# vfdev-5/interpolate-antialiasing

Hardware: AMD Instinct MI355X
Metric: Mpix/s (input pixels) antialiased bilinear 438x906->196x320, uint8 channels_last, PIL-exact (higher is better)
Workload: dtype u8; 1 GPU; uint8 channels_last [1024,3,438,906]->[196,320] bilinear antialias per GPU (BASELINE configs[1] batched), Pillow-exact integer arithmetic; batch_per_gpu=1024, global_batch=1024, variant=fused_u8_nhwc_pil_v3, parallelism=batch-shard x1, lib=interpolate_antialiasing_amd/csrc/libaa_interp.so

## Files before the change

### include/aa_interp.h

```cpp
#ifndef AA_INTERP_H
#define AA_INTERP_H

#include <stddef.h>
#include <stdint.h>

#ifdef __cplusplus
extern "C" {
#endif

#define AA_INTERP_ABI_VERSION 3

typedef void *aa_stream_t;

enum aa_status {
  AA_OK = 0,
  AA_ERR_BAD_FILTER = -1,
  AA_ERR_BAD_DTYPE = -2,
  AA_ERR_BAD_LAYOUT = -3,
  AA_ERR_BAD_SHAPE = -4,
  AA_ERR_NULL = -5,
  AA_ERR_WORKSPACE = -6,
  AA_ERR_KSIZE = -7,
  AA_ERR_HIP = -8,
  AA_ERR_NO_DEVICE = -9,
// ... 94 lines not shown
  int32_t out_layout;
  int32_t normalize;
  float mean[4];
  float std[4];
  uint32_t flags;
} aa_convert;
size_t aa_workspace_bytes_u8_to_f32(int layout, int64_t N, int64_t C, int64_t H, int64_t W, const aa_axis *ax_h, const aa_axis *ax_w,
                                    const aa_convert *cv);
int aa_resample_fwd_u8_to_f32(const void *in_dev, void *out_dev, void *workspace_dev, size_t workspace_bytes, int layout,
                              int64_t N, int64_t C, int64_t H, int64_t W, const aa_axis *ax_h, const aa_axis *ax_w,
                              const aa_convert *cv, aa_stream_t stream);

int aa_resample_bwd(const void *grad_out_dev, void *grad_in_dev, void *workspace_dev, size_t workspace_bytes, int dtype,
                    int layout, int64_t N, int64_t C, int64_t H, int64_t W, const aa_axis *tr_h, const aa_axis *tr_w,
                    aa_stream_t stream);
int aa_resample_bwd_atomic(const void *grad_out_dev, void *grad_in_dev, void *workspace_dev, size_t workspace_bytes,
                           int dtype, int layout, int64_t N, int64_t C, int64_t H, int64_t W, const aa_axis *ax_h,
                           const aa_axis *ax_w, aa_stream_t stream);
size_t aa_workspace_bytes_bwd(int dtype, int layout, int64_t N, int64_t C, int64_t H, int64_t W, int64_t oH, int64_t oW);

int aa_resample_axis_fwd(const void *in_dev, void *out_dev, int dtype, int64_t outer, int64_t in_size, int64_t inner,
                         const aa_axis *ax, aa_stream_t stream);

int aa_reduce_u8(const void *in_dev, void *out_dev, int layout, int64_t N, int64_t C, int64_t H, int64_t W, const int64_t *in_strides,
                 const int64_t *box, int fx, int fy, aa_stream_t stream);
int aa_premultiply_u8(const void *src_dev, void *dst_dev, int layout, int64_t N, int64_t C, int64_t H, int64_t W, aa_stream_t stream);
int aa_unpremultiply_u8(void *img_dev, int layout, int64_t N, int64_t C, int64_t H, int64_t W, aa_stream_t stream);

#define AA_MANY_FLIP_X 1
typedef struct aa_many_image {
  const void *data_dev;
  int64_t H, W;
  int64_t stride_row, stride_px, stride_ch;
  double box[4];
  int32_t has_box;
  int32_t flags;
} aa_many_image;
size_t aa_many_desc_bytes(int64_t n);
int aa_many_plan(int filter, int layout, int64_t n, int64_t C, int64_t oH, int64_t oW, const aa_many_image *images, void *desc_host,
                 size_t desc_bytes, size_t *workspace_bytes);
int aa_resample_many_u8(const void *desc_host, const void *desc_dev, int64_t n, int64_t C, int64_t oH, int64_t oW, int layout, void *out_dev,
                        void *workspace_dev, size_t workspace_bytes, aa_stream_t stream);
int aa_resample_many_u8_to_float(const void *desc_host, const void *desc_dev, int64_t n, int64_t C, int64_t oH, int64_t oW, int layout,
                                 void *out_dev, void *workspace_dev, size_t workspace_bytes, const aa_convert *cv, aa_stream_t stream);

int aa_probe_copy(const void *src_dev, void *dst_dev, size_t bytes, int form, aa_stream_t stream);

int aa_set_fused(int enabled);

int aa_set_store_form(int form);

int aa_set_plane_groups(int enabled);

const char *aa_last_variant(void);

#ifdef __cplusplus
}
#endif
#endif
```

### interpolate_antialiasing_amd/_lib.py

```python
from __future__ import annotations

import collections
import ctypes
import os

_HERE = os.path.dirname(os.path.abspath(__file__))
LIB_PATH = os.environ.get("AA_INTERP_LIB") or os.path.join(_HERE, "csrc", "libaa_interp.so")
HEADER_PATH = os.path.join(os.path.dirname(_HERE), "include", "aa_interp.h")

AA_OK = 0
FILTER_LINEAR, FILTER_CUBIC, FILTER_BOX, FILTER_HAMMING, FILTER_LANCZOS = 0, 1, 2, 3, 4
Filter = collections.namedtuple("Filter", "id name aliases support op")
FILTERS = (Filter(FILTER_LINEAR, "linear", ("bilinear",), 1.0, "linear"), Filter(FILTER_CUBIC, "cubic", ("bicubic",), 2.0, "cubic"),
           Filter(FILTER_BOX, "box", ("nearest",), 0.5, "nearest"), Filter(FILTER_HAMMING, "hamming", (), 1.0, "hamming"),
           Filter(FILTER_LANCZOS, "lanczos", (), 3.0, "lanczos"))
FILTER_NAMES = {f.id: f.name for f in FILTERS}


def by_filter_name(value) -> dict:
    return {n: value(f) for f in FILTERS for n in (f.name,) + f.aliases}


FILTER_IDS = by_filter_name(lambda f: f.id)
U8, F32, F64, F16, BF16 = 0, 1, 2, 3, 4
NCHW, NHWC = 0, 1
TABLE_PIL, TABLE_F32, TABLE_F64 = 0, 1, 2
ERR_BAD_DTYPE = -2
ERR_STRIDES = -10
FLAG_FAST = 1
FLAG_PREMUL_ALPHA = 2
FLAG_OUT_F16 = 4
FLAG_OUT_BF16 = 8

EXPORTS = (
    "aa_abi_version", "aa_strerror", "aa_device_count", "aa_table_ksize", "aa_table_bytes", "aa_table_build_bytes", "aa_table_build",
    "aa_table_transposed_ksize", "aa_table_transpose", "aa_table_query", "aa_table_query2", "aa_table_build2", "aa_workspace_bytes", "aa_resample_fwd",
    "aa_resample_bwd", "aa_resample_bwd_atomic", "aa_workspace_bytes_bwd", "aa_resample_axis_fwd", "aa_set_fused",
    "aa_last_variant", "aa_probe_copy", "aa_workspace_bytes_u8_to_f32", "aa_resample_fwd_u8_to_f32", "aa_set_store_form", "aa_set_plane_groups", "aa_resample_fwd_ex", "aa_resample_fwd_strided",
    "aa_workspace_bytes_ex", "aa_table_ksize_box", "aa_table_build_bytes_box", "aa_table_build_box", "aa_reduce_u8", "aa_premultiply_u8",
    "aa_unpremultiply_u8", "aa_many_desc_bytes", "aa_many_plan", "aa_resample_many_u8", "aa_resample_many_u8_to_float",
)


class TableHeader(ctypes.Structure):
    _fields_ = [
        ("magic", ctypes.c_int32), ("filter", ctypes.c_int32), ("kind", ctypes.c_int32), ("in_size", ctypes.c_int32),
        ("out_size", ctypes.c_int32), ("ksize", ctypes.c_int32), ("align_corners", ctypes.c_int32),
        ("max_taps", ctypes.c_int32), ("transposed", ctypes.c_int32), ("scatter_off", ctypes.c_int32),
        ("scatter_ksize", ctypes.c_int32), ("scatter_max", ctypes.c_int32), ("span64p1", ctypes.c_int32), ("span4p1", ctypes.c_int32), ("gather_off", ctypes.c_int32), ("reserved", ctypes.c_int32 * 1),
    ]


class Axis(ctypes.Structure):
    _fields_ = [
        ("table_dev", ctypes.c_void_p), ("in_size", ctypes.c_int32), ("out_size", ctypes.c_int32),
        ("ksize", ctypes.c_int32), ("max_taps", ctypes.c_int32), ("kind", ctypes.c_int32), ("filter", ctypes.c_int32),
        ("scatter_off", ctypes.c_int32), ("scatter_ksize", ctypes.c_int32), ("scatter_max", ctypes.c_int32),
        ("span64p1", ctypes.c_int32), ("span4p1", ctypes.c_int32), ("gather_off", ctypes.c_int32), ("reserved", ctypes.c_int32 * 2),
    ]


class Convert(ctypes.Structure):
    _fields_ = [("out_layout", ctypes.c_int32), ("normalize", ctypes.c_int32), ("mean", ctypes.c_float * 4),
                ("std", ctypes.c_float * 4), ("flags", ctypes.c_uint32)]


class ManyImage(ctypes.Structure):
    _fields_ = [("data_dev", ctypes.c_void_p), ("H", ctypes.c_int64), ("W", ctypes.c_int64), ("stride_row", ctypes.c_int64),
                ("stride_px", ctypes.c_int64), ("stride_ch", ctypes.c_int64), ("box", ctypes.c_double * 4), ("has_box", ctypes.c_int32),
                ("flags", ctypes.c_int32)]


class ManyHeader(ctypes.Structure):
    _fields_ = [("magic", ctypes.c_int32), ("n", ctypes.c_int32), ("C", ctypes.c_int32), ("oH", ctypes.c_int32), ("oW", ctypes.c_int32),
                ("filter", ctypes.c_int32), ("layout", ctypes.c_int32), ("reserved0", ctypes.c_int32), ("hunits", ctypes.c_int64),
                ("ws_bytes", ctypes.c_int64), ("reserved", ctypes.c_int64 * 2)]


class ManyItem(ctypes.Structure):
    _fields_ = [("src", ctypes.c_void_p), ("row_stride", ctypes.c_int64), ("plane_stride", ctypes.c_int64), ("tab_h", ctypes.c_int64),
                ("tab_w", ctypes.c_int64), ("inter", ctypes.c_int64), ("in0_h", ctypes.c_double), ("in1_h", ctypes.c_double),
                ("in0_w", ctypes.c_double), ("in1_w", ctypes.c_double), ("oy", ctypes.c_int32), ("hull_h", ctypes.c_int32),
                ("ox", ctypes.c_int32), ("hull_w", ctypes.c_int32), ("ksize_h", ctypes.c_int32), ("ksize_w", ctypes.c_int32),
                ("box_on", ctypes.c_int32), ("reserved", ctypes.c_int32)]


MANY_FLIP_X = 1
MANY_STRIP = 64


def many_desc_view(buf, n: int):
# ... 47 lines not shown
    L.aa_table_build2.restype = i32
    L.aa_workspace_bytes.argtypes = [i32, i32, i64, i64, i64, i64, i64, i64, ax, ax]
    L.aa_workspace_bytes.restype = sz
    L.aa_workspace_bytes_ex.argtypes = [i32, i32, i64, i64, i64, i64, i64, i64, ax, ax, ctypes.c_uint]
    L.aa_workspace_bytes_ex.restype = sz
    L.aa_resample_fwd.argtypes = [vp, vp, vp, sz, i32, i32, i64, i64, i64, i64, ax, ax, vp]
    L.aa_resample_fwd.restype = i32
    L.aa_resample_fwd_ex.argtypes = [vp, vp, vp, sz, i32, i32, i64, i64, i64, i64, ax, ax, ctypes.c_uint, vp]
    L.aa_resample_fwd_ex.restype = i32
    L.aa_resample_fwd_strided.argtypes = [vp, vp, i32, i32, i64, i64, i64, i64, ctypes.POINTER(ctypes.c_int64), ax, ax, ctypes.c_uint, vp]
    L.aa_resample_fwd_strided.restype = i32
    L.aa_resample_bwd.argtypes = [vp, vp, vp, sz, i32, i32, i64, i64, i64, i64, ax, ax, vp]
    L.aa_resample_bwd.restype = i32
    L.aa_resample_bwd_atomic.argtypes = [vp, vp, vp, sz, i32, i32, i64, i64, i64, i64, ax, ax, vp]
    L.aa_resample_bwd_atomic.restype = i32
    L.aa_workspace_bytes_bwd.argtypes = [i32, i32, i64, i64, i64, i64, i64, i64]
    L.aa_workspace_bytes_bwd.restype = sz
    L.aa_resample_axis_fwd.argtypes = [vp, vp, i32, i64, i64, i64, ax, vp]
    L.aa_resample_axis_fwd.restype = i32
    L.aa_last_variant.restype = ctypes.c_char_p
    cvp = ctypes.POINTER(Convert)
    L.aa_workspace_bytes_u8_to_f32.argtypes = [i32, i64, i64, i64, i64, ax, ax, cvp]
    L.aa_workspace_bytes_u8_to_f32.restype = sz
    L.aa_resample_fwd_u8_to_f32.argtypes = [vp, vp, vp, sz, i32, i64, i64, i64, i64, ax, ax, cvp, vp]
    L.aa_resample_fwd_u8_to_f32.restype = i32
    L.aa_probe_copy.argtypes = [vp, vp, sz, i32, vp]
    L.aa_probe_copy.restype = i32
    L.aa_table_ksize_box.argtypes = [i32, i32, i64, i64, dbl, dbl]
    L.aa_table_ksize_box.restype = i32
    L.aa_table_build_bytes_box.argtypes = [i32, i32, i64, i64, dbl, dbl]
    L.aa_table_build_bytes_box.restype = sz
    L.aa_table_build_box.argtypes = [i32, i32, i64, i64, i64, dbl, dbl, vp, sz, i64, i64, i64, dbl, dbl, vp, sz, vp]
    L.aa_table_build_box.restype = i32
    L.aa_reduce_u8.argtypes = [vp, vp, i32, i64, i64, i64, i64, ctypes.POINTER(ctypes.c_int64), ctypes.POINTER(ctypes.c_int64), i32, i32, vp]
    L.aa_reduce_u8.restype = i32
    L.aa_premultiply_u8.argtypes = [vp, vp, i32, i64, i64, i64, i64, vp]
    L.aa_premultiply_u8.restype = i32
    L.aa_unpremultiply_u8.argtypes = [vp, i32, i64, i64, i64, i64, vp]
    L.aa_unpremultiply_u8.restype = i32
    L.aa_many_desc_bytes.argtypes = [i64]
    L.aa_many_desc_bytes.restype = sz
    L.aa_many_plan.argtypes = [i32, i32, i64, i64, i64, i64, ctypes.POINTER(ManyImage), vp, sz, ctypes.POINTER(sz)]
    L.aa_many_plan.restype = i32
    L.aa_resample_many_u8.argtypes = [vp, vp, i64, i64, i64, i64, i32, vp, vp, sz, vp]
    L.aa_resample_many_u8.restype = i32
    L.aa_resample_many_u8_to_float.argtypes = [vp, vp, i64, i64, i64, i64, i32, vp, vp, sz, cvp, vp]
    L.aa_resample_many_u8_to_float.restype = i32
    L.aa_set_fused.argtypes = [i32]
    L.aa_set_fused.restype = i32
    L.aa_set_store_form.argtypes = [i32]
    L.aa_set_store_form.restype = i32
    L.aa_set_plane_groups.argtypes = [i32]
    L.aa_set_plane_groups.restype = i32
    if L.aa_abi_version() != 3:
        raise AAInterpError("libaa_interp.so ABI version mismatch")
    _lib = L
    return L


def strerror(rc: int) -> str:
    return load().aa_strerror(rc).decode()


def check(rc: int, what: str = "") -> None:
    if rc < 0:
        msg = f"{what}: {strerror(rc)} (aa_status {rc})" if what else f"{strerror(rc)} (aa_status {rc})"
        if rc == ERR_BAD_DTYPE:
            raise NotImplementedError(msg)
        raise AAInterpError(msg)


fused_epoch = 0


def set_fused(enabled: int) -> int:
    global fused_epoch
    fused_epoch += 1
    return int(load().aa_set_fused(int(enabled)))


def set_store_form(form: int) -> int:
    return int(load().aa_set_store_form(int(form)))


def set_plane_groups(enabled: int) -> int:
    return int(load().aa_set_plane_groups(int(enabled)))


def last_variant() -> str:
    return load().aa_last_variant().decode()


KERNEL_SOURCES = {
    "fused_u8_nhwc_pil_v3": ("aa_fused_u8_v3_impl.h", "aa_fused_u8_v3.hip", "aa_fused_u8_v3_unit.hip", "aa_fused_u8_v3_list.h", "aa_common.h"),
    "fused_u8_nhwc_pil": ("aa_fused_u8.hip", "aa_common.h"),
    "fused_u8_planar_pil_v3": ("aa_fused_u8_v3_impl.h", "aa_fused_u8_v3.hip", "aa_fused_u8_v3_unit.hip", "aa_fused_u8_v3_list.h", "aa_common.h"),
}


def source_fingerprint(variant: str):
    import hashlib

    names = KERNEL_SOURCES.get(variant)
    if not names:
        return None
    h = hashlib.sha256()
    for n in names:
        with open(os.path.join(_HERE, "csrc", n), "rb") as f:
            h.update(n.encode() + b"\0" + f.read())
    return h.hexdigest()[:12]
```

### interpolate_antialiasing_amd/csrc/aa_api.hip

```cpp

#include <math.h>
#include <string.h>

#include "aa_box.h"
#include "aa_many.h"
#include "aa_plan.h"
#include "aa_reduce.h"

int g_aa_store_form = -1;
int g_aa_plane_groups = 1;

namespace {

thread_local const char *g_last_variant = "none";
int g_fused_enabled = 1;

int interp_size_of(int filter) { return aa_filter_valid(filter) ? aa_filter_info(filter).interp_size : -1; }

double scale_for(int kind, int64_t in_size, int64_t out_size, int align_corners, double scale_opt) {
  if (kind == AA_TABLE_F32) {
    if (align_corners) return out_size > 1 ? (double)((float)(in_size - 1) / (float)(out_size - 1)) : 0.0;
    if (scale_opt > 0.) return (double)(float)(1.0 / scale_opt);
    return (double)((float)in_size / (float)out_size);
  }
  if (align_corners) return out_size > 1 ? (double)(in_size - 1) / (double)(out_size - 1) : 0.0;
  if (scale_opt > 0.) return 1.0 / scale_opt;
  return (double)in_size / (double)out_size;
}

int ksize_for(int filter, int kind, double scale) {
  const int interp_size = interp_size_of(filter);
  if (kind == AA_TABLE_PIL) {
    const double fs = aa_filter_info(filter).support;
    const double filterscale = scale < 1.0 ? 1.0 : scale;
    return (int)ceil(fs * filterscale) * 2 + 1;
  }
  if (kind == AA_TABLE_F32) {
    const float s = (float)scale;
    const float support = (s >= 1.0) ? (float)((interp_size * 0.5) * s) : (float)(interp_size * 0.5);
    return (int)ceilf(support) * 2 + 1;
  }
  const double support = (scale >= 1.0) ? (interp_size * 0.5) * scale : interp_size * 0.5;
  return (int)ceilf((float)support) * 2 + 1;
}

bool valid_kind(int kind) { return kind == AA_TABLE_PIL || kind == AA_TABLE_F32 || kind == AA_TABLE_F64; }

int check_axis(const aa_axis *a, int64_t in_size) {
  if (!a || !a->table_dev) return AA_ERR_NULL;
  if (a->in_size != in_size || a->out_size <= 0 || a->ksize <= 0) return AA_ERR_BAD_SHAPE;
  if (a->ksize > AA_MAX_KSIZE) return AA_ERR_KSIZE;
  if (!valid_kind(a->kind)) return AA_ERR_BAD_DTYPE;
  return AA_OK;
}

int check_dtype_kind(int dtype, int kh, int kw) {
  if (kh != kw) return AA_ERR_BAD_DTYPE;
  if (dtype == AA_F32 && kh == AA_TABLE_F32) return AA_OK;
  if (dtype == AA_F64 && kh == AA_TABLE_F64) return AA_OK;
  if (dtype == AA_U8 && (kh == AA_TABLE_PIL || kh == AA_TABLE_F32)) return AA_OK;
  if ((dtype == AA_F16 || dtype == AA_BF16) && kh == AA_TABLE_F32) return AA_OK;
  return AA_ERR_BAD_DTYPE;
}
// ... 550 lines not shown
    g_last_variant = "empty";
    return AA_OK;
  }
  if (!grad_out_dev || !grad_in_dev) return AA_ERR_NULL;
  const size_t need = aa_workspace_bytes_bwd(dtype, layout, N, C, H, W, ax_h->out_size, ax_w->out_size);
  if (!workspace_dev || workspace_bytes < need) return AA_ERR_WORKSPACE;
  AAProblem q = problem(dtype, layout, N, C, H, W, ax_h->out_size, ax_w->out_size, *ax_h, *ax_w, 0u);
  q.in = grad_out_dev; q.out = grad_in_dev; q.ws = workspace_dev; q.ws_bytes = workspace_bytes;
  q.stream = (hipStream_t)stream;
  rc = aa_launch_bwd_atomic(q);
  if (rc == AA_OK) g_last_variant = "bwd_scatter_atomics";
  return rc;
}

int aa_resample_axis_fwd(const void *in_dev, void *out_dev, int dtype, int64_t outer, int64_t in_size, int64_t inner,
                         const aa_axis *ax, aa_stream_t stream) {
  if (dtype < AA_U8 || dtype > AA_BF16) return AA_ERR_BAD_DTYPE;
  if (outer < 0 || in_size <= 0 || inner <= 0) return AA_ERR_BAD_SHAPE;
  int rc = check_axis(ax, in_size);
  if (rc != AA_OK) return rc;
  if (dtype == AA_U8 && ax->kind != AA_TABLE_PIL) return AA_ERR_BAD_DTYPE;
  rc = check_dtype_kind(dtype, ax->kind, ax->kind);
  if (rc != AA_OK) return rc;
  if (outer == 0) return AA_OK;
  if (!in_dev || !out_dev) return AA_ERR_NULL;
  g_last_variant = "generic_axis";
  return aa_launch_axis_fwd(in_dev, out_dev, dtype, outer, in_size, inner, *ax, (hipStream_t)stream);
}

int aa_probe_copy(const void *src_dev, void *dst_dev, size_t bytes, int form, aa_stream_t stream) {
  if (!src_dev || !dst_dev) return AA_ERR_NULL;
  if ((((uintptr_t)src_dev | (uintptr_t)dst_dev) & 15) != 0 || form < 0 || form > 5) return AA_ERR_BAD_SHAPE;
  return aa_launch_probe_copy(src_dev, dst_dev, bytes, form, (hipStream_t)stream);
}

int aa_set_fused(int enabled) {
  const int prev = g_fused_enabled;
  g_fused_enabled = (enabled < 0 || enabled > 2) ? 1 : enabled;
  return prev;
}

int aa_set_store_form(int form) {
  const int prev = g_aa_store_form;
  g_aa_store_form = (form < -1 || form > 1) ? -1 : form;
  return prev;
}

int aa_set_plane_groups(int enabled) {
  const int prev = g_aa_plane_groups;
  g_aa_plane_groups = enabled ? 1 : 0;
  return prev;
}

const char *aa_last_variant(void) { return g_last_variant; }

}
```

### interpolate_antialiasing_amd/csrc/aa_common.h

```cpp
#pragma once

#include <hip/hip_runtime.h>
#include <stdint.h>

#include "../../include/aa_interp.h"

#define AA_TABLE_MAGIC 0x42544141
#define AA_MAX_KSIZE 4096

struct AAFilterInfo {
  double support;
  int interp_size;
  bool nonneg;
};
__host__ __device__ inline bool aa_filter_valid(int filter) { return filter >= AA_FILTER_LINEAR && filter <= AA_FILTER_LANCZOS; }
__host__ __device__ inline AAFilterInfo aa_filter_info(int filter) {
  switch (filter) {
    case AA_FILTER_LINEAR: return {1.0, 2, true};
    case AA_FILTER_CUBIC: return {2.0, 4, false};
    case AA_FILTER_BOX: return {0.5, 1, true};
    case AA_FILTER_HAMMING: return {1.0, 2, true};
    case AA_FILTER_LANCZOS: return {3.0, 6, false};
    default: return {0.0, -1, false};
  }
}
__host__ __device__ inline bool aa_filters_nonneg(int filter_a, int filter_b) {
  return aa_filter_info(filter_a).nonneg && aa_filter_info(filter_b).nonneg;
}

__host__ __device__ inline size_t aa_align16(size_t x) { return (x + 15) & ~(size_t)15; }
__host__ __device__ inline size_t aa_weight_elem_bytes(int kind) { return kind == AA_TABLE_F64 ? 8 : 4; }
__host__ __device__ inline size_t aa_table_xmin_off() { return sizeof(aa_table_header); }
__host__ __device__ inline size_t aa_table_xsize_off(int64_t out) { return sizeof(aa_table_header) + 4 * (size_t)out; }
__host__ __device__ inline size_t aa_table_w_off(int64_t out) {
  return aa_align16(sizeof(aa_table_header) + 8 * (size_t)out);
}
__host__ __device__ inline size_t aa_table_weights_end(int kind, int64_t out, int ksize) {
  return aa_align16(aa_table_w_off(out) + (size_t)out * (size_t)ksize * aa_weight_elem_bytes(kind));
}
__host__ __device__ inline size_t aa_table_gather_bytes(int kind, int64_t out) { return (kind == AA_TABLE_F32 || kind == AA_TABLE_PIL) ? 32 * (size_t)out : 0; }
__host__ __device__ inline size_t aa_table_total_bytes(int kind, int64_t out, int ksize) {
  return aa_table_weights_end(kind, out, ksize) + aa_table_gather_bytes(kind, out);
}

template <typename WT>
struct TableView {
  const int32_t *xmin;
  const int32_t *xsize;
  const WT *w;
  int ksize;
};

template <typename WT>
__host__ __device__ inline TableView<WT> make_table_view(const void *table, int out_size, int ksize) {
  const char *p = (const char *)table;
  TableView<WT> v;
  v.xmin = (const int32_t *)(p + aa_table_xmin_off());
  v.xsize = (const int32_t *)(p + aa_table_xsize_off(out_size));
  v.w = (const WT *)(p + aa_table_w_off(out_size));
  v.ksize = ksize;
  return v;
}

#include <stdlib.h>
#ifdef AA_V2_TUNING
inline const char *aa_knob(const char *name) { return getenv(name); }
#else
inline const char *aa_knob(const char *) { return nullptr; }
#endif
extern int g_aa_store_form;
extern int g_aa_plane_groups;

#define AA_HIP_CHECK_LAUNCH()                 \
  do {                                        \
    if (hipGetLastError() != hipSuccess) return AA_ERR_HIP; \
  } while (0)

__host__ __device__ inline size_t aa_table_scatter_pitch(int kind) { return kind == AA_TABLE_F64 ? 64 : 32; }
__host__ __device__ inline size_t aa_table_scatter_bytes(int kind, int64_t in_size, int scatter_ksize) {
  return scatter_ksize > 0 ? aa_table_scatter_pitch(kind) * ((size_t)in_size + 1) : 0;
}
int aa_launch_table_transpose(const aa_table_header &h, const void *table_dev, void *tr_dev, int tr_ksize,
                              hipStream_t stream);

struct AAProblem {
  const void *in;
  void *out;
  void *ws;
  size_t ws_bytes;
  int dtype, layout;
  int64_t N, C, H, W, oH, oW;
  aa_axis ah, aw;
  hipStream_t stream;
  int out_f32 = 0;
  int out_elem = AA_F32;
  int out_layout = AA_NCHW;
  int normalize = 0;
  float mean[4] = {0.f, 0.f, 0.f, 0.f};
  float std[4] = {1.f, 1.f, 1.f, 1.f};
  int64_t in_row_pitch = 0, in_img_pitch = 0;
  int fast = 0;
  int alpha = 0;
};

int aa_launch_generic_fwd(const AAProblem &p, const char **variant);
int aa_launch_axis_fwd(const void *in, void *out, int dtype, int64_t outer, int64_t in_size, int64_t inner, const aa_axis &ax,
                       hipStream_t stream);
size_t aa_generic_workspace_bytes(int dtype, int kind_w, int64_t N, int64_t C, int64_t H, int64_t oW);
int aa_launch_generic_convert(const AAProblem &p, const char **variant);
int aa_launch_premul_u8(const void *src, void *dst, int layout, int64_t N, int64_t C, int64_t H, int64_t W, hipStream_t stream);
int aa_launch_unpremul_u8(void *img, int layout, int64_t N, int64_t C, int64_t H, int64_t W, hipStream_t stream);
inline int aa_strip_span_px(const aa_axis &aw, int tw) { return aw.span64p1 > 0 ? aw.span64p1 + tw : -1; }
inline int aa_strip_span_px32(const aa_axis &aw, int tw) {
  if (aw.span64p1 <= 0 || aw.span4p1 <= 0) return -1;
  const int by4 = 11 * (aw.span4p1 - 1) + 1;
  return (by4 < aw.span64p1 ? by4 : aw.span64p1) + tw;
}
inline int aa_strip_span_px16(const aa_axis &aw, int tw) {
  if (aw.span64p1 <= 0 || aw.span4p1 <= 0) return -1;
  const int by4 = 5 * (aw.span4p1 - 1) + 1;
  return (by4 < aw.span64p1 ? by4 : aw.span64p1) + tw;
}
inline bool aa_grid_fits(int64_t units) { return units > 0 && units <= (int64_t)0x7FFFFFFF / 64 - 8; }
int aa_device_cu_count();
// ... 28 lines not shown
```

### interpolate_antialiasing_amd/csrc/aa_fused_u8_v3_impl.h

```cpp

#pragma once
#include <math.h>
#include <stdio.h>
#include <stdlib.h>

#include <type_traits>

#include "aa_alpha.h"
#include "aa_plan.h"

#ifndef AA_V3_ABL
#define AA_V3_ABL 0
#endif

#ifndef AA_V3_AUX
#define AA_V3_AUX 0
#endif

#ifndef AA_V3_PRIO
#define AA_V3_PRIO 0
#endif
#ifndef AA_V3_DMA_EARLY
#define AA_V3_DMA_EARLY 0
#endif

#ifndef AA_V3_BURST
#define AA_V3_BURST 1
#endif

#ifndef AA_V3_F32OUT_AUX
#define AA_V3_F32OUT_AUX 0
#endif

#ifndef AA_V3_FLT_FAST
#define AA_V3_FLT_FAST 0
#endif

#ifndef AA_V3_UNALIGNED
#define AA_V3_UNALIGNED 0
#endif

struct FusedU8V3Params {
  int H, W, oH, oW;
  int ksize_w, ksize_h;
  int ybands, nstrips;
  int strips_per_block;
  int strip_w;
  int nseg;
  int seg_bytes;
  int sc_off;
  int gather_off;
  int in_mis;
  unsigned long long img_in_bytes, img_out_bytes, total_in_bytes, total_out_bytes;
  long long n_images;
  int spb_forced;
  int outm, normalize, cin;
  float mean[4], std[4];
  unsigned row_pitch;
  int fast;
  int byte_store;
  unsigned long long plane_in_bytes, plane_out_bytes;
  long long pl_planes;
  int out16, pair_store;
};

namespace {

typedef __attribute__((address_space(3))) void lds_void;

#ifndef AA_V3_STORE_AUX
#define AA_V3_STORE_AUX 2
#endif
constexpr int kStoreAuxInterleaved = AA_V3_STORE_AUX;



__device__ inline unsigned pack4_clip8(int a0, int a1, int a2, int a3) {
  unsigned d;
  asm("v_ashr_pk_u8_i32 %0, %1, %2, 22\n\tv_ashr_pk_u8_i32 %0, %3, %4, 22 op_sel:[0,0,0,1]"
      : "=&v"(d)
      : "v"(a0), "v"(a1), "v"(a2), "v"(a3));
  return d;
}

__device__ inline unsigned pack2_bf16(float lo, float hi) {
  unsigned d;
  asm("v_cvt_pk_bf16_f32 %0, %1, %2" : "=v"(d) : "v"(lo), "v"(hi));
  return d;
}
__device__ inline unsigned pack2_f16(float lo, float hi) {
  typedef _Float16 half2_t __attribute__((ext_vector_type(2)));
  const half2_t t = {(_Float16)lo, (_Float16)hi};
  return __builtin_bit_cast(unsigned, t);
}

__device__ inline float right_neighbour(float x) {
  return __int_as_float(__builtin_amdgcn_update_dpp(__float_as_int(x), __float_as_int(x), 0xF5 , 0xF, 0xF, false));
}

__device__ inline int clip8_int(int acc) {
  acc >>= 22;
  return acc < 0 ? 0 : (acc > 255 ? 255 : acc);
}

__device__ inline void wait_vmcnt(int n) {
  if (n >= 12) { asm volatile("s_waitcnt vmcnt(12)" ::: "memory"); return; }
  if (n >= 8) { asm volatile("s_waitcnt vmcnt(8)" ::: "memory"); return; }
  if (n >= 6) { asm volatile("s_waitcnt vmcnt(6)" ::: "memory"); return; }
  if (n >= 4) { asm volatile("s_waitcnt vmcnt(4)" ::: "memory"); return; }
  if (n >= 3) { asm volatile("s_waitcnt vmcnt(3)" ::: "memory"); return; }
  if (n >= 2) { asm volatile("s_waitcnt vmcnt(2)" ::: "memory"); return; }
  if (n >= 1) { asm volatile("s_waitcnt vmcnt(1)" ::: "memory"); return; }
  asm volatile("s_waitcnt vmcnt(0)" ::: "memory");
}

#ifndef AA_V3_WAVES_PER_EU
#define AA_V3_WAVES_PER_EU 0
#endif
#if AA_V3_WAVES_PER_EU
#define AA_V3_OCC __attribute__((amdgpu_waves_per_eu(AA_V3_WAVES_PER_EU, AA_V3_WAVES_PER_EU)))
#else
#define AA_V3_OCC
#endif
template <int C, int TW, int G, bool TWO_DMA, int MAXC, bool NONNEG, bool PERIODIC, bool FLT = false, int UPK = 0, int PL = 0, int SP = 1,
          bool ALPHA = false, bool O16 = false>
__global__ void __launch_bounds__(512) AA_V3_OCC
fused_u8_nhwc_v3_kernel(const uint8_t *__restrict__ in, uint8_t *__restrict__ out, const char *__restrict__ tab_w,
                        const char *__restrict__ tab_h, const FusedU8V3Params p) {
  static_assert(PL == 0 || (PL == C && !PERIODIC && UPK == 0 && !TWO_DMA), "plane groups: shrinking heights, fixed stage layout");
  static_assert(SP == 1 || (SP == 4 && !FLT && !PERIODIC && UPK == 0 && PL == 0), "split windows: integer arithmetic, shrinking heights");
  static_assert(!ALPHA || (C == 4 && !FLT && PL == 0), "premultiplied alpha: Pillow arithmetic, 4 interleaved channels");
  static_assert(!O16 || (FLT && SP == 1), "16-bit float output: float arithmetic");
  constexpr int PLN = PL > 0 ? PL : 1;
  constexpr int CB = PL > 0 ? 1 : C;
  constexpr int NV1 = (CB * TW + 3) / 4;
  constexpr int ND1 = NV1 + 1;
  constexpr int NV = PLN * NV1, ND = PLN * ND1;
  struct SA { unsigned s[PLN]; };
  constexpr int PL_SLOT = 1024, PL_PIECES = 21, PL_PLANE = PL_PIECES * 16;
  extern __shared__ __attribute__((aligned(16))) uint8_t lds[];

  const int lane = threadIdx.x & 63;
  const int wv = __builtin_amdgcn_readfirstlane(threadIdx.x >> 6);
  const int sgroups = (p.nstrips + p.strips_per_block - 1) / p.strips_per_block;
  const int xcd = blockIdx.x & 7, k = blockIdx.x >> 3;
  const int strip = (k % sgroups) * p.strips_per_block + wv;
  const long long grp = (long long)(k / sgroups) * 8 + xcd;
  if (grp >= p.n_images * p.ybands) return;
  if (strip >= p.nstrips) return;
  const bool full_group = (k % sgroups + 1) * p.strips_per_block <= p.nstrips;
  const int yb = (int)(grp % p.ybands);
  const int n = (int)(grp / p.ybands);
  const int ox0 = strip * p.strip_w;
  const int bw = min(p.strip_w, p.oW - ox0);
  const int oy0 = (int)((long long)yb * p.oH / p.ybands);
  const int oy1 = (int)((long long)(yb + 1) * p.oH / p.ybands);

  const int32_t *__restrict__ xmin_w = (const int32_t *)(tab_w + aa_table_xmin_off());
  const int32_t *__restrict__ xsize_w = (const int32_t *)(tab_w + aa_table_xsize_off(p.oW));
  const int32_t *__restrict__ kw = (const int32_t *)(tab_w + aa_table_w_off(p.oW));
  const int32_t *__restrict__ ymin_h = (const int32_t *)(tab_h + aa_table_xmin_off());
  const int32_t *__restrict__ ysize_h = (const int32_t *)(tab_h + aa_table_xsize_off(p.oH));
  const int32_t *__restrict__ sc_rec = (const int32_t *)(tab_h + p.sc_off);
  const int32_t *__restrict__ g_rec = (const int32_t *)(tab_h + p.gather_off);

  const int r_begin = __builtin_amdgcn_readfirstlane(ymin_h[oy0]);
  const int ylm = __builtin_amdgcn_readfirstlane(ymin_h[oy1 - 1]);
  const int yls = __builtin_amdgcn_readfirstlane(ysize_h[oy1 - 1]);
  const int r_stop = ylm + (yls > 1 ? yls : 1);
  const int n_rows = r_stop - r_begin;
  const int n_groups = (n_rows + G - 1) / G;

  const int sp_px = SP > 1 ? lane / SP : lane;
  const int sp_part = SP > 1 ? lane % SP : 0;
  const bool active = sp_px < bw;
  const int ox = ox0 + (active ? sp_px : 0);
  const int xm = xmin_w[ox];
  int xs = xsize_w[ox];
  xs = xs > 1 ? xs : 1;
  int lead = xm + TW * SP - p.W;
  lead = lead > 0 ? lead : 0;
  const int start = xm - lead + sp_part * TW;
  const int acc_init = (SP > 1 && sp_part != 0) ? 0 : 1 << 21;
  int wreg[TW];
#pragma unroll
  for (int j = 0; j < TW; j++) {
    const int src = sp_part * TW + j - lead;
    int w = (src >= 0 && src < xs && src < p.ksize_w) ? kw[(size_t)ox * p.ksize_w + src] : 0;
    wreg[j] = FLT ? w : (w << 8) >> 8;
  }
  asm volatile("s_waitcnt vmcnt(0)" ::: "memory");
  const int seg_first = __builtin_amdgcn_readfirstlane(start * CB);
  const int c_l = start * CB - seg_first;

  const unsigned long long img_off = (unsigned long long)p.in_mis + (unsigned long long)n * p.img_in_bytes;
  const unsigned long long base_off = img_off & ~15ull;
  unsigned long long remaining = p.total_in_bytes - base_off;
  if constexpr (PL == 0) remaining = (remaining + 3ull) & ~3ull;
  if (remaining > 0xFFFFFFFCull) remaining = 0xFFFFFFFCull;
  const __amdgpu_buffer_rsrc_t rsrc =
      __builtin_amdgcn_make_buffer_rsrc((void *)(in + base_off), 0, (unsigned)remaining, 0x00020000);
  const unsigned row_bytes = p.row_pitch;
  const int lds_base = PL > 0 ? wv * G * PL_SLOT : wv * G * p.seg_bytes;
  const unsigned lane_lds = (unsigned)(lds_base + c_l);
  unsigned pl_voff = 0;
  bool pl_dma_lane = false;
  if constexpr (PL > 0) {
    const int pc = lane / PL_PIECES, piece = lane - pc * PL_PIECES;
    pl_voff = (unsigned)pc * (unsigned)p.plane_in_bytes + (unsigned)piece * 16u;
// ... 495 lines not shown
        } else {
          realign(d1, sa1, v);
          __builtin_amdgcn_sched_barrier(0);
          sc0 = load_scatter(r + 1);
          sa0 = fetch(a + row_bytes, (i + 1) % G, d0);
          __builtin_amdgcn_sched_barrier(0);
          if (AA_V3_DMA_EARLY) { dma(a + (unsigned)G * row_bytes, i); __builtin_amdgcn_sched_barrier(0); }
          row_step(v, sc1, steady_tag);
        }
        if (!AA_V3_DMA_EARLY) {
          if constexpr (AA_V3_BURST == 1) {
            dma(a + (unsigned)G * row_bytes, i);
          } else if ((i % AA_V3_BURST) == AA_V3_BURST - 1) {
#pragma unroll
            for (int b = AA_V3_BURST - 1; b >= 0; b--) dma(a + (unsigned)(G - b) * row_bytes, i - b);
          }
        }
        a += row_bytes;
        r++;
        __builtin_amdgcn_sched_barrier(0);
      }
    };
    if (UPK == 0 && x0 + 2 * G <= n_rows) {
      if (steady) unrolled_group(std::true_type{});
      else unrolled_group(std::false_type{});
    } else {
      for (int i = 0; i < G; i++) {
        const int x = x0 + i;
        if (x >= n_rows) break;
        if (x + 1 < n_rows) {
          if constexpr (UPK > 0) {
            const int my_idx = __builtin_amdgcn_readlane(idxv, __builtin_amdgcn_readfirstlane((i + 1) % G));
            wait_vmcnt(vm_issued - my_idx);
          } else {
            int younger = n_rows - 1 - (x + 1);
            younger = younger < G - 2 ? younger : G - 2;
            wait_vmcnt(younger * dma_per_row);
          }
          if (PL > 0 && r + 1 == pl_fix_row) pl_patch_last((i + 1) % G);
          if ((i & 1) == 0) { sc1 = load_scatter(r + 1); sa1 = fetch(a + row_bytes, (i + 1) % G, d1, false); }
          else { sc0 = load_scatter(r + 1); sa0 = fetch(a + row_bytes, (i + 1) % G, d0, false); }
        }
        unsigned v[NV];
        if ((i & 1) == 0) { realign(d0, sa0, v); row_step(v, sc0, std::false_type{}); }
        else { realign(d1, sa1, v); row_step(v, sc1, std::false_type{}); }
        if (x + G < n_rows) dma(a + (unsigned)G * row_bytes, i);
        a += row_bytes;
        r++;
      }
    }
  }
}

int pick_ybands(int64_t items_per_band, double slots, int taps_h, int64_t H, int64_t oH) {
  const int64_t max_yb = oH / 8 > 1 ? oH / 8 : 1;
  int64_t ybands = 1;
  double best = 1e30;
  for (int64_t yb = 1; yb <= max_yb && yb <= 64; yb++) {
    const double rounds = (double)items_per_band * yb / slots;
    const double eff = rounds / ceil(rounds);
    const double halo = 1.0 + (double)(yb - 1) * taps_h / (double)H;
    const double cost = halo / eff;
    if (cost < best - 1e-9) {
      best = cost;
      ybands = yb;
    }
  }
  if (const char *e = aa_knob("AA_FUSED_YBANDS")) {
    const int64_t v = atoll(e);
    if (v >= 1 && v <= max_yb) ybands = v;
  }
  return (int)ybands;
}

template <int C, int TW, int G, int MAXC, bool TWO, bool NONNEG, bool PERIODIC, bool FLT = false, int UPK = 0, int PL = 0, int SP = 1,
          bool ALPHA = false, bool O16 = false>
int launch_k(FusedU8V3Params p, const AAProblem &q, size_t lds) {
  auto kern = fused_u8_nhwc_v3_kernel<C, TW, G, TWO, MAXC, NONNEG, PERIODIC, FLT, UPK, PL, SP, ALPHA, O16>;
  auto resident = [&](int s) {
    int nb = aa_resident_blocks(kern, 64 * s, lds * s);
    if (nb <= 0) nb = 16 / s;
    return nb < 1 ? 1 : nb;
  };
  int spb = p.strips_per_block;
  if (spb > 1 && !p.spb_forced && resident(1) > resident(spb) * spb) spb = 1;
  p.strips_per_block = spb;
  const int sgroups = (p.nstrips + spb - 1) / spb;
  const size_t lds_blk = lds * spb;
  const int taps_h = q.ah.max_taps > 0 ? q.ah.max_taps : q.ah.ksize;
  p.ybands = pick_ybands(p.n_images * sgroups, (double)aa_device_cu_count() * resident(spb), taps_h, q.H, q.oH);
  if (aa_knob("AA_V3_DEBUG"))
    fprintf(stderr, "[aa v3] strips %d spb %d (resident(1) %d, resident(%d) %d) ybands %d lds/strip %zu images %lld\n", p.nstrips, spb,
            resident(1), p.nstrips <= 8 ? p.nstrips : 4, resident(p.nstrips <= 8 ? p.nstrips : 4), p.ybands, lds, (long long)p.n_images);
  const int64_t groups8 = (p.n_images * (int64_t)p.ybands + 7) / 8 * 8;
  const int64_t grid = groups8 * sgroups;
  if (grid > 0x7FFFFFFF) return 0;
  hipLaunchKernelGGL(kern, dim3((unsigned)grid), dim3(64 * spb), lds_blk,
                     q.stream, (const uint8_t *)q.in - p.in_mis, (uint8_t *)q.out, (const char *)q.aw.table_dev,
                     (const char *)q.ah.table_dev, p);
  AA_HIP_CHECK_LAUNCH();
  return 1;
}

int round_tw(int taps) {
  const int opts[] = {2, 4, 6, 8, 12, 16, 24, 34};
  for (int o : opts)
    if (taps <= o) return o;
  return 0;
}

}

enum V3Route {
#define V3_ROUTE(route, ...) V3_##route,
#include "aa_fused_u8_v3_list.h"
};
enum V3Arith { V3_PIL = 1, V3_FLT = 2, V3_BOTH = 3 };
constexpr bool v3_route_has_out16(int route) { return route == V3_NARROW || route == V3_UP || route == V3_PLANES; }
```

Measured before the change: 1.423 million Mpix/s.

## Add tiered per-image row-band schedule for fused u8 v3 kernel

Replaces the single uniform y-band count with a schedule of up to four tiers, where later images can be split into more row bands. The goal is to shrink the idle tail of the last wave while limiting vertical halo overhead. The default model has max_tiers=1, so it picks a uniform band count through the same whole-rounds cost as before. Forced tiers can be set through a new API or environment knob. The kernel now decodes image and band from the schedule with a few extra compares per block.

```diff
diff --git a/include/aa_interp.h b/include/aa_interp.h
--- a/include/aa_interp.h
+++ b/include/aa_interp.h
@@ -170,6 +170,8 @@
 
 int aa_set_plane_groups(int enabled);
 
+int aa_set_band_schedule(int ntiers, const int *bands, const int *images_permille);
+
 const char *aa_last_variant(void);
 
 #ifdef __cplusplus
diff --git a/interpolate_antialiasing_amd/_lib.py b/interpolate_antialiasing_amd/_lib.py
--- a/interpolate_antialiasing_amd/_lib.py
+++ b/interpolate_antialiasing_amd/_lib.py
@@ -36,7 +36,7 @@
     "aa_abi_version", "aa_strerror", "aa_device_count", "aa_table_ksize", "aa_table_bytes", "aa_table_build_bytes", "aa_table_build",
     "aa_table_transposed_ksize", "aa_table_transpose", "aa_table_query", "aa_table_query2", "aa_table_build2", "aa_workspace_bytes", "aa_resample_fwd",
     "aa_resample_bwd", "aa_resample_bwd_atomic", "aa_workspace_bytes_bwd", "aa_resample_axis_fwd", "aa_set_fused",
-    "aa_last_variant", "aa_probe_copy", "aa_workspace_bytes_u8_to_f32", "aa_resample_fwd_u8_to_f32", "aa_set_store_form", "aa_set_plane_groups", "aa_resample_fwd_ex", "aa_resample_fwd_strided",
+    "aa_last_variant", "aa_probe_copy", "aa_workspace_bytes_u8_to_f32", "aa_resample_fwd_u8_to_f32", "aa_set_store_form", "aa_set_plane_groups", "aa_set_band_schedule", "aa_resample_fwd_ex", "aa_resample_fwd_strided",
     "aa_workspace_bytes_ex", "aa_table_ksize_box", "aa_table_build_bytes_box", "aa_table_build_box", "aa_reduce_u8", "aa_premultiply_u8",
     "aa_unpremultiply_u8", "aa_many_desc_bytes", "aa_many_plan", "aa_resample_many_u8", "aa_resample_many_u8_to_float",
 )
@@ -190,6 +190,8 @@
     L.aa_set_store_form.restype = i32
     L.aa_set_plane_groups.argtypes = [i32]
     L.aa_set_plane_groups.restype = i32
+    L.aa_set_band_schedule.argtypes = [i32, ctypes.POINTER(i32), ctypes.POINTER(i32)]
+    L.aa_set_band_schedule.restype = i32
     if L.aa_abi_version() != 3:
         raise AAInterpError("libaa_interp.so ABI version mismatch")
     _lib = L
@@ -225,14 +227,23 @@
     return int(load().aa_set_plane_groups(int(enabled)))
 
 
+def set_band_schedule(bands=(), images_permille=()) -> None:
+    bands, pm = [int(b) for b in bands], [int(v) for v in images_permille]
+    if bands and len(pm) != len(bands) - 1:
+        raise ValueError("images_permille holds one value per tier but the last")
+    b = (ctypes.c_int32 * max(len(bands), 1))(*bands)
+    m = (ctypes.c_int32 * max(len(pm), 1))(*pm)
+    check(load().aa_set_band_schedule(len(bands), b, m), "aa_set_band_schedule")
+
+
 def last_variant() -> str:
     return load().aa_last_variant().decode()
 
 
 KERNEL_SOURCES = {
-    "fused_u8_nhwc_pil_v3": ("aa_fused_u8_v3_impl.h", "aa_fused_u8_v3.hip", "aa_fused_u8_v3_unit.hip", "aa_fused_u8_v3_list.h", "aa_common.h"),
+    "fused_u8_nhwc_pil_v3": ("aa_fused_u8_v3_impl.h", "aa_band_schedule.h", "aa_fused_u8_v3.hip", "aa_fused_u8_v3_unit.hip", "aa_fused_u8_v3_list.h", "aa_common.h"),
     "fused_u8_nhwc_pil": ("aa_fused_u8.hip", "aa_common.h"),
-    "fused_u8_planar_pil_v3": ("aa_fused_u8_v3_impl.h", "aa_fused_u8_v3.hip", "aa_fused_u8_v3_unit.hip", "aa_fused_u8_v3_list.h", "aa_common.h"),
+    "fused_u8_planar_pil_v3": ("aa_fused_u8_v3_impl.h", "aa_band_schedule.h", "aa_fused_u8_v3.hip", "aa_fused_u8_v3_unit.hip", "aa_fused_u8_v3_list.h", "aa_common.h"),
 }
 
 
diff --git a/interpolate_antialiasing_amd/csrc/aa_api.hip b/interpolate_antialiasing_amd/csrc/aa_api.hip
--- a/interpolate_antialiasing_amd/csrc/aa_api.hip
+++ b/interpolate_antialiasing_amd/csrc/aa_api.hip
@@ -9,6 +9,7 @@
 
 int g_aa_store_form = -1;
 int g_aa_plane_groups = 1;
+AABandForce g_aa_band_force = {};
 
 namespace {
 
@@ -665,6 +666,18 @@
   return prev;
 }
 
+int aa_set_band_schedule(int ntiers, const int *bands, const int *images_permille) {
+  if (ntiers < 0 || ntiers > 4 || (ntiers > 0 && !bands) || (ntiers > 1 && !images_permille)) return AA_ERR_BAD_SHAPE;
+  AABandForce f = {};
+  f.ntiers = ntiers;
+  for (int t = 0; t < ntiers; t++) {
+    f.bands[t] = bands[t];
+    f.permille[t] = t < ntiers - 1 ? images_permille[t] : 0;
+  }
+  g_aa_band_force = f;
+  return 0;
+}
+
 const char *aa_last_variant(void) { return g_last_variant; }
 
 }
diff --git a/interpolate_antialiasing_amd/csrc/aa_band_schedule.h b/interpolate_antialiasing_amd/csrc/aa_band_schedule.h
--- /dev/null
+++ b/interpolate_antialiasing_amd/csrc/aa_band_schedule.h
@@ -0,0 +1,160 @@
+#pragma once
+#include <math.h>
+
+#if defined(__HIPCC__) || defined(__CUDACC__)
+#define AA_BS_HD __host__ __device__
+#else
+#define AA_BS_HD
+#endif
+
+enum { AA_BAND_TIERS = 4, AA_BAND_MAX = 64 };
+
+struct AABandSchedule {
+  int ntiers;
+  int bands[AA_BAND_TIERS];
+  long long img0[AA_BAND_TIERS + 1];
+  long long grp0[AA_BAND_TIERS + 1];
+};
+
+AA_BS_HD inline void aa_band_decode(const AABandSchedule &s, long long grp, long long *image, int *band, int *bands) {
+  const unsigned g = (unsigned)grp, g1 = (unsigned)s.grp0[1], g2 = (unsigned)s.grp0[2], g3 = (unsigned)s.grp0[3];
+  const bool t1 = g >= g1, t2 = g >= g2, t3 = g >= g3;
+  const unsigned nb = (unsigned)(t3 ? s.bands[3] : t2 ? s.bands[2] : t1 ? s.bands[1] : s.bands[0]);
+  const unsigned g0 = t3 ? g3 : t2 ? g2 : t1 ? g1 : 0u;
+  const unsigned i0 = t3 ? (unsigned)s.img0[3] : t2 ? (unsigned)s.img0[2] : t1 ? (unsigned)s.img0[1] : 0u;
+  const unsigned local = g - g0;
+  const unsigned q = local / nb;
+  *image = (long long)(i0 + q);
+  *band = (int)(local - q * nb);
+  *bands = (int)nb;
+}
+
+AA_BS_HD inline void aa_band_rows(int band, int bands, int oH, int *oy0, int *oy1) {
+  *oy0 = (int)((long long)band * oH / bands);
+  *oy1 = (int)((long long)(band + 1) * oH / bands);
+}
+
+
+inline int aa_band_clamp(long long bands, int oH) {
+  const int max_b = oH / 8 < 1 ? 1 : oH / 8 > AA_BAND_MAX ? AA_BAND_MAX : oH / 8;
+  return bands < 1 ? 1 : bands > max_b ? max_b : (int)bands;
+}
+
+inline void aa_band_schedule_fill(AABandSchedule *s, int ntiers, const int *bands, const long long *nimg) {
+  int n = 0;
+  long long img = 0, grp = 0;
+  s->img0[0] = s->grp0[0] = 0;
+  for (int t = 0; t < ntiers && n < AA_BAND_TIERS; t++) {
+    if (nimg[t] <= 0) continue;
+    s->bands[n] = bands[t];
+    img += nimg[t];
+    grp += nimg[t] * bands[t];
+    n++;
+    s->img0[n] = img;
+    s->grp0[n] = grp;
+  }
+  if (n == 0) s->bands[n++] = 1, s->img0[1] = s->grp0[1] = 0;
+  s->ntiers = n;
+  for (int t = n; t < AA_BAND_TIERS; t++) {
+    s->bands[t] = s->bands[n - 1];
+    s->img0[t + 1] = img;
+    s->grp0[t + 1] = grp;
+  }
+}
+
+inline void aa_band_schedule_uniform(AABandSchedule *s, long long N, int bands, int oH) {
+  const int b = aa_band_clamp(bands, oH);
+  aa_band_schedule_fill(s, 1, &b, &N);
+}
+
+inline void aa_band_schedule_forced(AABandSchedule *s, long long N, int oH, int ntiers, const int *bands, const int *permille) {
+  int b[AA_BAND_TIERS];
+  long long n[AA_BAND_TIERS], left = N;
+  ntiers = ntiers < 1 ? 1 : ntiers > AA_BAND_TIERS ? AA_BAND_TIERS : ntiers;
+  for (int t = 0; t < ntiers; t++) {
+    b[t] = aa_band_clamp(bands[t], oH);
+    if (t > 0 && b[t] < b[t - 1]) b[t] = b[t - 1];
+    long long want = left;
+    if (t < ntiers - 1) {
+      const long long pm = permille[t] < 0 ? 0 : permille[t];
+      want = (N * pm + 500) / 1000;
+      if (want > left) want = left;
+    }
+    n[t] = want;
+    left -= want;
+  }
+  aa_band_schedule_fill(s, ntiers, b, n);
+}
+
+struct AABandModel {
+  double h_eq;
+  double tier_scale;
+  double min_rounds;
+  int max_tiers;
+};
+constexpr AABandModel kAABandModelTapered = {6.6, 1.0, 2.0, 4};
+constexpr AABandModel kAABandModel = {6.6, 1.0, 2.0, 1};
+
+inline int aa_band_whole_rounds(long long items_per_band, double slots, int taps_h, long long H, int oH) {
+  const int max_b = aa_band_clamp(AA_BAND_MAX, oH);
+  int bands = 1;
+  double best = 1e30;
+  for (int b = 1; b <= max_b; b++) {
+    const double rounds = (double)items_per_band * b / slots;
+    const double eff = rounds / ceil(rounds);
+    const double halo = 1.0 + (double)(b - 1) * taps_h / (double)H;
+    const double cost = halo / eff;
+    if (cost < best - 1e-9) best = cost, bands = b;
+  }
+  return bands;
+}
+
+inline void aa_band_schedule_build(AABandSchedule *s, long long N, int sgroups, double slots, int taps_h, long long H, int oH,
+                                   const AABandModel &m = kAABandModel) {
+  const int max_b = aa_band_clamp(AA_BAND_MAX, oH);
+  if (m.max_tiers <= 1) {
+    aa_band_schedule_uniform(s, N, aa_band_whole_rounds(N * sgroups, slots, taps_h, H, oH), oH);
+    return;
+  }
+  const double per_slot = (double)sgroups / slots;
+  auto D = [&](int b) { return (double)H / b + m.h_eq; };
+  auto img_work = [&](int b) { return per_slot * b * D(b); };
+  int best_nt = 0, best_b[AA_BAND_TIERS];
+  long long best_n[AA_BAND_TIERS];
+  double best = 1e300;
+  for (int b0 = 1; b0 <= 8 && b0 <= max_b; b0++) {
+    int b[AA_BAND_TIERS] = {b0, 0, 0, 0};
+    long long n[AA_BAND_TIERS] = {N, 0, 0, 0};
+    for (int nt = 1; nt <= AA_BAND_TIERS && nt <= m.max_tiers; nt++) {
+      if (nt > 1) {
+        b[nt - 1] = 2 * b[nt - 2] > max_b ? max_b : 2 * b[nt - 2];
+        if (b[nt - 1] == b[nt - 2]) break;
+        const double idle = 0.5 * (D(b[nt - 2]) - D(b[nt - 1]));
+        n[nt - 1] = (long long)(m.tier_scale * idle / img_work(b[nt - 1]) + 0.5);
+        n[0] -= n[nt - 1];
+      }
+      if (n[0] <= 0 || (double)n[0] * b0 * per_slot < m.min_rounds) break;
+      double cost = 0.5 * D(b[nt - 1]);
+      for (int t = 0; t < nt; t++) cost += n[t] * img_work(b[t]);
+      if (cost < best - 1e-9) {
+        best = cost, best_nt = nt;
+        for (int t = 0; t < nt; t++) best_b[t] = b[t], best_n[t] = n[t];
+      }
+    }
+  }
+  if (best_nt <= 1) {
+    double bu = m.h_eq > 0 && N > 0 ? H / (2.0 * m.h_eq * N * per_slot) : 1.0;
+    int lo = 1;
+    while (lo < max_b && (double)(lo + 1) * (lo + 1) <= bu) lo++;
+    for (int b = lo; b <= lo + 1 && b <= max_b; b++) {
+      if ((double)N * b * per_slot < m.min_rounds) continue;
+      const double cost = N * img_work(b) + 0.5 * D(b);
+      if (cost < best - 1e-9) best = cost, best_nt = 1, best_b[0] = b, best_n[0] = N;
+    }
+  }
+  if (best_nt == 0) {
+    aa_band_schedule_uniform(s, N, aa_band_whole_rounds(N * sgroups, slots, taps_h, H, oH), oH);
+    return;
+  }
+  aa_band_schedule_fill(s, best_nt, best_b, best_n);
+}
diff --git a/interpolate_antialiasing_amd/csrc/aa_common.h b/interpolate_antialiasing_amd/csrc/aa_common.h
--- a/interpolate_antialiasing_amd/csrc/aa_common.h
+++ b/interpolate_antialiasing_amd/csrc/aa_common.h
@@ -70,6 +70,8 @@
 #endif
 extern int g_aa_store_form;
 extern int g_aa_plane_groups;
+struct AABandForce { int ntiers, bands[4], permille[4]; };
+extern AABandForce g_aa_band_force;
 
 #define AA_HIP_CHECK_LAUNCH()                 \
   do {                                        \
diff --git a/interpolate_antialiasing_amd/csrc/aa_fused_u8_v3_impl.h b/interpolate_antialiasing_amd/csrc/aa_fused_u8_v3_impl.h
--- a/interpolate_antialiasing_amd/csrc/aa_fused_u8_v3_impl.h
+++ b/interpolate_antialiasing_amd/csrc/aa_fused_u8_v3_impl.h
@@ -7,6 +7,7 @@
 #include <type_traits>
 
 #include "aa_alpha.h"
+#include "aa_band_schedule.h"
 #include "aa_plan.h"
 
 #ifndef AA_V3_ABL
@@ -62,6 +63,7 @@
   unsigned long long plane_in_bytes, plane_out_bytes;
   long long pl_planes;
   int out16, pair_store;
+  AABandSchedule sched;
 };
 
 namespace {
@@ -146,15 +148,16 @@
   const int xcd = blockIdx.x & 7, k = blockIdx.x >> 3;
   const int strip = (k % sgroups) * p.strips_per_block + wv;
   const long long grp = (long long)(k / sgroups) * 8 + xcd;
-  if (grp >= p.n_images * p.ybands) return;
+  if (grp >= p.sched.grp0[AA_BAND_TIERS]) return;
   if (strip >= p.nstrips) return;
   const bool full_group = (k % sgroups + 1) * p.strips_per_block <= p.nstrips;
-  const int yb = (int)(grp % p.ybands);
-  const int n = (int)(grp / p.ybands);
+  long long image;
+  int yb, nbands, oy0, oy1;
+  aa_band_decode(p.sched, grp, &image, &yb, &nbands);
+  aa_band_rows(yb, nbands, p.oH, &oy0, &oy1);
+  const int n = (int)image;
   const int ox0 = strip * p.strip_w;
   const int bw = min(p.strip_w, p.oW - ox0);
-  const int oy0 = (int)((long long)yb * p.oH / p.ybands);
-  const int oy1 = (int)((long long)(yb + 1) * p.oH / p.ybands);
 
   const int32_t *__restrict__ xmin_w = (const int32_t *)(tab_w + aa_table_xmin_off());
   const int32_t *__restrict__ xsize_w = (const int32_t *)(tab_w + aa_table_xsize_off(p.oW));
@@ -756,25 +759,28 @@
   }
 }
 
-int pick_ybands(int64_t items_per_band, double slots, int taps_h, int64_t H, int64_t oH) {
-  const int64_t max_yb = oH / 8 > 1 ? oH / 8 : 1;
-  int64_t ybands = 1;
-  double best = 1e30;
-  for (int64_t yb = 1; yb <= max_yb && yb <= 64; yb++) {
-    const double rounds = (double)items_per_band * yb / slots;
-    const double eff = rounds / ceil(rounds);
-    const double halo = 1.0 + (double)(yb - 1) * taps_h / (double)H;
-    const double cost = halo / eff;
-    if (cost < best - 1e-9) {
-      best = cost;
-      ybands = yb;
+void v3_band_schedule(AABandSchedule *s, long long n_images, int sgroups, double slots, int taps_h, int64_t H, int64_t oH) {
+  AABandForce f = g_aa_band_force;
+  if (const char *e = aa_knob("AA_V3_SCHED")) {
+    f.ntiers = 0;
+    while (f.ntiers < AA_BAND_TIERS && *e) {
+      char *end;
+      f.bands[f.ntiers] = (int)strtol(e, &end, 10);
+      if (end == e) break;
+      e = end;
+      f.permille[f.ntiers] = 0;
+      if (*e == ':') { f.permille[f.ntiers] = (int)strtol(e + 1, &end, 10); e = end; }
+      f.ntiers++;
+      if (*e == ',') e++;
     }
   }
   if (const char *e = aa_knob("AA_FUSED_YBANDS")) {
     const int64_t v = atoll(e);
-    if (v >= 1 && v <= max_yb) ybands = v;
-  }
-  return (int)ybands;
+    const int64_t max_yb = oH / 8 > 1 ? oH / 8 : 1;
+    if (v >= 1 && v <= max_yb) { f.ntiers = 1; f.bands[0] = (int)v; }
+  }
+  if (f.ntiers > 0) aa_band_schedule_forced(s, n_images, (int)oH, f.ntiers, f.bands, f.permille);
+  else aa_band_schedule_build(s, n_images, sgroups, slots, taps_h, H, (int)oH);
 }
 
 template <int C, int TW, int G, int MAXC, bool TWO, bool NONNEG, bool PERIODIC, bool FLT = false, int UPK = 0, int PL = 0, int SP = 1,
@@ -792,11 +798,13 @@
   const int sgroups = (p.nstrips + spb - 1) / spb;
   const size_t lds_blk = lds * spb;
   const int taps_h = q.ah.max_taps > 0 ? q.ah.max_taps : q.ah.ksize;
-  p.ybands = pick_ybands(p.n_images * sgroups, (double)aa_device_cu_count() * resident(spb), taps_h, q.H, q.oH);
+  v3_band_schedule(&p.sched, p.n_images, sgroups, (double)aa_device_cu_count() * resident(spb), taps_h, q.H, q.oH);
+  p.ybands = p.sched.bands[0];
   if (aa_knob("AA_V3_DEBUG"))
-    fprintf(stderr, "[aa v3] strips %d spb %d (resident(1) %d, resident(%d) %d) ybands %d lds/strip %zu images %lld\n", p.nstrips, spb,
-            resident(1), p.nstrips <= 8 ? p.nstrips : 4, resident(p.nstrips <= 8 ? p.nstrips : 4), p.ybands, lds, (long long)p.n_images);
-  const int64_t groups8 = (p.n_images * (int64_t)p.ybands + 7) / 8 * 8;
+    fprintf(stderr, "[aa v3] strips %d spb %d (resident(1) %d, resident(%d) %d) tiers %d bands %d/%d/%d/%d from image 0/%lld/%lld/%lld lds/strip %zu images %lld\n",
+            p.nstrips, spb, resident(1), p.nstrips <= 8 ? p.nstrips : 4, resident(p.nstrips <= 8 ? p.nstrips : 4), p.sched.ntiers, p.sched.bands[0],
+            p.sched.bands[1], p.sched.bands[2], p.sched.bands[3], p.sched.img0[1], p.sched.img0[2], p.sched.img0[3], lds, (long long)p.n_images);
+  const int64_t groups8 = (p.sched.grp0[AA_BAND_TIERS] + 7) / 8 * 8;
   const int64_t grid = groups8 * sgroups;
   if (grid > 0x7FFFFFFF) return 0;
   hipLaunchKernelGGL(kern, dim3((unsigned)grid), dim3(64 * spb), lds_blk,
```

New measurement: 1.421 million Mpix/s. No clear change (-0.1%).
